# zyc00/Point-SAM

Measured on AMD Instinct MI355X. Metric: point-clouds/sec (encode+1-prompt decode), higher is better.
Workload: dtype f32 (fp32 in/out/accumulate; large GEMMs as row-scaled 2-way fp16 split x 3 MFMA products, fp32-grade error)

## Files before the change

include/pointsam_hip.h:

```cpp
#ifndef POINTSAM_HIP_H
#define POINTSAM_HIP_H

#include <stddef.h>
#include <stdint.h>

#ifdef __cplusplus
extern "C" {
#endif

typedef struct ihipStream_t* psam_stream_t;

#define PSAM_OK 0
#define PSAM_EINVAL (-1)
#define PSAM_EALIGN (-2)
#define PSAM_EWORKSPACE (-3)

#define PSAM_ACT_NONE 0
#define PSAM_ACT_GELU 1
#define PSAM_ACT_RELU 2
#define PSAM_ACT_SWIGLU 3

int32_t psam_version(void);
const char* psam_last_error_string(void);

// ... 59 lines not shown
void psam_gemm_f16x3p_force_splitk_fixup(int32_t mode);
#ifdef PSAM_BUILD_EXPERIMENTS
void psam_gemm_f16x3p_force_continuous(int32_t mode);
#endif
#define PSAM_COUNTER_BYTES 65536
void psam_attention_f16x3_force_keysplit(int32_t mode);
int32_t psam_attention_f16x3_last_instance(void);
int32_t psam_attention_f16x3_last_keysplit(void);
int32_t psam_attention_f32_last_instance(void);
#ifdef PSAM_BUILD_EXPERIMENTS
void psam_twoway_decoder_force_fork(int32_t mode);
#endif
int32_t psam_gemm_f16x3p_fused_row_ln(int32_t N);
typedef struct {
    float* out_scale; float out_k1, out_k2; int32_t pack_out;
    float* stats; int32_t stat_cols;
    const float* ln_mean; const float* ln_rstd; const float* ln_c;
    float* gmax_out; int64_t gmax_ld; int32_t gmax_k; int32_t no_store;
    const float* row_ln_g; const float* row_ln_b; float row_ln_eps;
    const float* hyper; float* masks; int32_t hyper_c; int32_t hyper_rows;
    int64_t hyper_pstride;
    float* splitk_ws; int64_t splitk_plane; int32_t splitk;
    const float* out_bound;
    int32_t* counters;
} psam_gemm_fuse_t;
int32_t psam_gemm_f16x3p_splitk(int32_t M, int32_t N, int32_t K, int32_t act);
int32_t psam_gemm_f16x3p_hyper_planes(int32_t N, int32_t with_row_ln);
int32_t psam_sum_planes(const float* parts, int32_t P, int64_t pstride, int64_t count, float* out, psam_stream_t stream);
int32_t psam_gemm_f16x3p_stat_segs(int32_t N);
int32_t psam_gemm_f16x3p_ex(const void* A, int64_t lda, const float* scaleA, const void* W, int64_t ldw, const float* scaleW, float* C, int64_t ldc,
                            const float* bias, const float* residual, int64_t ldr, const float* rowbias, int64_t ldrb, int32_t rowgroup, int32_t M,
                            int32_t N, int32_t K, float alpha, int32_t act, const psam_gemm_fuse_t* fuse, psam_stream_t stream);
int32_t psam_ln_stats_finalize(const float* stats, int32_t rows, int32_t segs, int32_t cols, float eps, float* mean, float* rstd, psam_stream_t stream);
int32_t psam_scale_pack_rows_g8(const float* X, int64_t ldx, int32_t rows, int32_t K, void* P, int64_t ldp, float* scale, psam_stream_t stream);
int32_t psam_linear(const float* x, int64_t ldx, const float* W, int64_t ldw, const float* bias, const float* residual, int64_t ldr, float* y,
                    int64_t ldy, int32_t M, int32_t N, int32_t K, int32_t act, psam_stream_t stream);
void psam_gemm_bf16x6_force_config(int32_t cfg);
void psam_gemm_force_config(int32_t cfg);

int32_t psam_layernorm(const float* x, int64_t ldx, const float* res, int64_t ldr, const float* w, const float* b, float* y, int64_t ldy,
                       int64_t rows, int32_t cols, float eps, int32_t act, psam_stream_t stream);
int32_t psam_layernorm_ex(const float* x, int64_t ldx, const float* res, int64_t ldr, const float* w, const float* b, float* y, int64_t ldy,
                          int64_t rows, int32_t cols, float eps, int32_t act, float* row_scale, int32_t pack, psam_stream_t stream);
int32_t psam_layernorm_ex2(const float* x, int64_t ldx, const float* res, int64_t ldr, const float* w, const float* b, float* y, int64_t ldy,
                           int64_t rows, int32_t cols, float eps, int32_t act, float* row_scale, int32_t pack, float* row_bound, float c2,
                           float c1, float c0, psam_stream_t stream);
int32_t psam_layernorm_rs(const float* x, int64_t ldx, const float* res, int64_t ldr, const float* w, const float* b, float* y, int64_t ldy,
                          int64_t rows, int32_t cols, float eps, int32_t act, float* row_scale, psam_stream_t stream);
int32_t psam_layernorm_last_instance(void);

int32_t psam_swiglu_ln(const float* gx, int64_t ldg, int32_t xoff, const float* w, const float* b, float* out, int64_t ldo, int64_t rows,
                       int32_t H, float eps, psam_stream_t stream);
int32_t psam_swiglu_ln_last_instance(void);

int32_t psam_attention_f32(const float* q, int64_t ldq, int64_t sq, const float* k, int64_t ldk, int64_t sk, const float* v, int64_t ldv,
                           int64_t sv, float* o, int64_t ldo, int64_t so, int32_t B, int32_t H, int32_t Lq, int32_t Lk, int32_t hd,
                           float scale, psam_stream_t stream);
int32_t psam_attention_f16x3(const float* q, int64_t ldq, int64_t sq, const float* k, int64_t ldk, int64_t sk, const float* v, int64_t ldv,
                           int64_t sv, float* o, int64_t ldo, int64_t so, int32_t B, int32_t H, int32_t Lq, int32_t Lk, int32_t hd,
                           float scale, psam_stream_t stream);
int32_t psam_attention_f16x3_ex(const float* q, int64_t ldq, int64_t sq, const float* k, int64_t ldk, int64_t sk, const float* v, int64_t ldv,
                                int64_t sv, float* o, int64_t ldo, int64_t so, int32_t B, int32_t H, int32_t Lq, int32_t Lk, int32_t hd, float scale,
                                const float* a_scale, float k1, float k2, float* o_scale, psam_stream_t stream);
size_t psam_attention_f16x3_keysplit_ws_bytes(int32_t B, int32_t H, int32_t Lq, int32_t Lk, int32_t hd, int32_t max_keysplit);
int32_t psam_attention_f16x3_ex2(const float* q, int64_t ldq, int64_t sq, const float* k, int64_t ldk, int64_t sk, const float* v, int64_t ldv,
                                int64_t sv, float* o, int64_t ldo, int64_t so, int32_t B, int32_t H, int32_t Lq, int32_t Lk, int32_t hd, float scale,
// ... 291 lines not shown
```

point_sam_amd/_lib.py:

```python
import ctypes
import os

_HERE = os.path.dirname(os.path.abspath(__file__))
LIB_PATH = os.environ.get("PSAM_HIP_LIB") or os.path.join(_HERE, "csrc", "libpointsam_hip.so")

i32, i64, f32 = ctypes.c_int32, ctypes.c_int64, ctypes.c_float
ptr, size_t = ctypes.c_void_p, ctypes.c_size_t

SIGNATURES = {
    "psam_version": (i32, []),
    "psam_last_error_string": (ctypes.c_char_p, []),
    "psam_fps_workspace_bytes": (size_t, [i32, i32, i32]),
    "psam_fps_set_cooperative": (None, [i32]),
    "psam_fps_set_pruning": (None, [i32]),
    "psam_fps": (i32, [ptr, i32, i32, i32, ptr, ptr, ptr, size_t, ptr]),
    "psam_knn": (i32, [ptr, ptr, i32, i32, i32, i32, ptr, ptr]),
    "psam_fps_last_instance": (i32, []),
    "psam_fps_last_grid_x": (i32, []),
    "psam_knn_force_band": (None, [i32]),
    "psam_knn_last_instance": (i32, []),
    "psam_three_nn": (i32, [ptr, ptr, i32, i32, i32, f32, ptr, ptr, ptr]),
    "psam_group_gather": (i32, [ptr, ptr, ptr, ptr, i32, i32, i32, i32, i32, i32, ptr, ptr]),
    "psam_group_gather_r": (i32, [ptr, ptr, ptr, ptr, i32, i32, i32, i32, i32, i32, f32, ptr, ptr]),
    "psam_group_gather_ld": (i32, [ptr, ptr, ptr, ptr, i32, i32, i32, i32, i32, i32, f32, ptr, i64, ptr]),
    "psam_patch_l1": (i32, [ptr, ptr, ptr, ptr, ptr, ptr, ptr, ptr, f32, i32, i32, i32, i32, i32, i32, ptr, ptr]),
    "psam_patch_l1_r": (i32, [ptr, ptr, ptr, ptr, ptr, ptr, ptr, ptr, f32, i32, i32, i32, i32, i32, i32, f32, ptr, ptr]),
    "psam_patch_l1_ex": (i32, [ptr, ptr, ptr, ptr, ptr, ptr, ptr, ptr, ptr, f32, i32, i32, i32, i32, i32, i32, f32, ptr, ptr, ptr]),
    "psam_error_regions": (i32, [ptr, ptr, ptr, ptr, i64, ptr]),
    "psam_border_farthest_workspace_bytes": (size_t, [i32, i32]),
    "psam_border_farthest": (i32, [ptr, ptr, i32, i32, i32, ptr, ptr, ptr, size_t, ptr]),
    "psam_group_max": (i32, [ptr, i64, ptr, i64, i64, i32, i32, ptr]),
    "psam_gemm_f32": (i32, [ptr, i64, i64, i64, ptr, i64, i64, i64, ptr, i64, i64, i64, ptr, ptr, i64, i64, i64, ptr, i64, i32,
                            i32, i32, i32, i32, i32, f32, i32, ptr]),
    "psam_gemm_bf16x6": (i32, [ptr, i64, i64, i64, ptr, i64, i64, i64, ptr, i64, i64, i64, ptr, ptr, i64, i64, i64, ptr, i64, i32,
                               i32, i32, i32, i32, i32, f32, i32, ptr]),
    "psam_linear": (i32, [ptr, i64, ptr, i64, ptr, ptr, i64, ptr, i64, i32, i32, i32, i32, ptr]),
    "psam_gemm_force_config": (None, [i32]),
    "psam_gemm_bf16x6_force_config": (None, [i32]),
    "psam_row_scale_f16": (i32, [ptr, i64, i32, i32, ptr, ptr]),
    "psam_pack_rows_f16x2_g8": (i32, [ptr, i64, ptr, i32, i32, ptr, i64, ptr]),
    "psam_gemm_f16x3p": (i32, [ptr, i64, ptr, ptr, i64, ptr, ptr, i64, ptr, ptr, i64, ptr, i64, i32, i32, i32, i32, f32, i32, ptr]),
    "psam_gemm_f16x3p_force_config": (None, [i32]),
    "psam_gemm_f16x3p_last_config": (i32, []),
    "psam_gemm_f16x3p_last_splitk": (i32, []),
    "psam_gemm_f16x3p_force_epilogue": (None, [i32]),
    "psam_gemm_f16x3p_force_splitk_fixup": (None, [i32]),
    "psam_gemm_f16x3p_force_continuous": (None, [i32]),
    "psam_attention_f16x3_force_keysplit": (None, [i32]),
    "psam_attention_f16x3_last_instance": (i32, []),
    "psam_attention_f16x3_last_keysplit": (i32, []),
    "psam_attention_f32_last_instance": (i32, []),
    "psam_twoway_decoder_force_fork": (None, [i32]),
    "psam_attention_packed_force_variant": (None, [i32]),
    "psam_attention_packed_force_nw": (None, [i32]),
    "psam_attention_packed_last_instance": (i32, []),
    "psam_gemm_f16x3p_fused_row_ln": (i32, [i32]),
    "psam_gemm_f16x3p_stat_segs": (i32, [i32]),
    "psam_gemm_f16x3p_splitk": (i32, [i32, i32, i32, i32]),
    "psam_nn_group_feats": (i32, [ptr, ptr, ptr, ptr, ptr, i32, i32, i32, i32, i32, i32, ptr, i64, ptr]),
    "psam_scatter_amax": (i32, [ptr, i64, ptr, i64, i32, i64, i64, i32, ptr, i64, i32, ptr]),
    "psam_eva_block_prepared_bytes": (size_t, [i32, i32]),
    "psam_eva_block_prepare": (i32, [ptr, ptr, ptr, size_t, ptr]),
    "psam_eva_block_ws_bytes": (size_t, [i64, i32, i32]),
    "psam_eva_block": (i32, [ptr, ptr, ptr, i32, i32, ptr, size_t, ptr]),
    "psam_linear_skinny_multi": (i32, [ptr, i64, i64, i64, i32, i32, ptr]),
    "psam_linear_skinny_ln": (i32, [ptr, i64, ptr, i64, ptr, ptr, i64, ptr, ptr, f32, ptr, ptr, i64, i32, i32, i32, ptr, ptr]),
    "psam_linear_rows_multi": (i32, [ptr, i64, i64, i32, i32, i64, i64, i32, ptr]),
    "psam_linear_ln256": (i32, [ptr, i64, ptr, i64, ptr, ptr, i64, ptr, ptr, f32, ptr, i64, i64, i32, i32, ptr]),
    "psam_twoway_decoder_force_fast": (None, [i32]),
    "psam_scale_pack_rows_g8_add_dual": (i32, [ptr, i64, ptr, i64, i32, i32, i32, i32, ptr, ptr, ptr, ptr, i64, ptr]),
    "psam_mlp3_pair": (i32, [ptr, ptr, i32, ptr]),
    "psam_attention_small_force_split": (None, [i32]),
    "psam_attention_small_last_instance": (i32, []),
    "psam_layernorm_last_instance": (i32, []),
    "psam_swiglu_ln_last_instance": (i32, []),
    "psam_patch_l1_last_instance": (i32, []),
    "psam_interp3_last_instance": (i32, []),
    "psam_linear_skinny_ln_tmp_floats": (ctypes.c_size_t, [i32, i32]),
    "psam_scale_pack_rows_g8_add": (i32, [ptr, i64, ptr, i64, i32, i32, i32, i32, ptr, i64, ptr, ptr]),
    "psam_eva_gelu_block_prepared_bytes": (size_t, [i32, i32]),
    "psam_eva_gelu_block_prepare": (i32, [ptr, ptr, ptr, size_t, ptr]),
    "psam_eva_gelu_block_ws_bytes": (size_t, [i64, i32, i32]),
    "psam_eva_gelu_block": (i32, [ptr, ptr, ptr, i32, i32, ptr, size_t, ptr, ptr]),
    "psam_patch_encoder_prepared_bytes": (size_t, [i32, i32, i32]),
    "psam_patch_encoder_prepare": (i32, [ptr, ptr, ptr, size_t, ptr]),
    "psam_patch_encoder_ws_bytes": (size_t, [i64, i64, i32, i32]),
    "psam_patch_encoder": (i32, [ptr, ptr, ptr, ptr, ptr, ptr, ptr, i32, i32, i32, i32, i32, i32, f32, ptr, ptr, size_t, ptr]),
    "psam_upscale_masks_prepared_bytes": (size_t, [i32]),
    "psam_upscale_masks_prepare": (i32, [ptr, ptr, ptr, size_t, ptr]),
# ... 211 lines not shown
```

point_sam_amd/build.py:

```python
import os
import subprocess
import sys
from concurrent.futures import ThreadPoolExecutor

CSRC = os.path.join(os.path.dirname(os.path.abspath(__file__)), "csrc")
LIB = os.path.join(CSRC, "libpointsam_hip.so")
HIPCC = os.environ.get("HIPCC", "/opt/rocm/bin/hipcc")
ARCH = "gfx950"
COMMON = ["--offload-arch=" + ARCH, "-O3", "-std=c++17", "-fPIC", "-fvisibility=hidden", "-Wall", "-Wno-unused-function"]
EXPERIMENTS = os.environ.get("PSAM_BUILD_EXPERIMENTS", "0") == "1"
SOURCES = [
    ("tokenizer.hip", ["-ffp-contract=off"]),
    ("gemm.hip", []),
    ("gemm_split.hip", []),
    ("gemm_f16x3p.hip", []),
    ("gemm_f16x3pp.hip", []),
    ("attention.hip", []),
    ("rowops.hip", []),
    ("blocks.hip", []),
    ("masks.hip", []),
    ("scene.hip", ["-ffp-contract=off"]),
    ("regions.hip", ["-ffp-contract=off"]),
    ("crops.hip", ["-ffp-contract=off"]),
    ("scene_interp.hip", ["-ffp-contract=off"]),
    ("transfer.hip", ["-ffp-contract=off", "-fno-slp-vectorize"]),
    ("align.hip", ["-ffp-contract=off", "-fno-slp-vectorize"]),
    ("views.hip", ["-ffp-contract=off", "-fno-slp-vectorize"]),
    ("frames.hip", ["-ffp-contract=off", "-fno-slp-vectorize"]),
    ("fusion.hip", ["-ffp-contract=off", "-fno-slp-vectorize"]),
    ("geometry.hip", ["-ffp-contract=off", "-fno-slp-vectorize"]),
    ("error.cpp", ["-x", "hip"]),
] + ([("experiments/gemm_f16x3q.hip", ["-I" + CSRC]), ("experiments/gemm_f16x3s.hip", ["-I" + CSRC]), ("experiments/gemm_f16x3c.hip", ["-I" + CSRC]),
        ("experiments/twoway.hip", ["-I" + CSRC])] if EXPERIMENTS else [])
if EXPERIMENTS:
    COMMON = COMMON + ["-DPSAM_BUILD_EXPERIMENTS"]
FLAGS_STAMP = os.path.join(CSRC, ".build_flags")
PROBE_SRC = os.path.join(CSRC, "probe", "mfma_probe.hip")
PROBE_LIB = os.path.join(CSRC, "probe", "libpsam_probe.so")


def _stale(out, deps):
    return not os.path.exists(out) or any(os.path.getmtime(d) > os.path.getmtime(out) for d in deps)


def build_library(force: bool = False, verbose: bool = False) -> str:
    hdrs = [os.path.join(CSRC, f) for f in sorted(os.listdir(CSRC)) if f.endswith(".h")]
    hdrs.append(os.path.join(os.path.dirname(os.path.dirname(CSRC)), "include", "pointsam_hip.h"))
    flags = " ".join(COMMON)
    if (open(FLAGS_STAMP).read() != flags) if os.path.exists(FLAGS_STAMP) else EXPERIMENTS:
# ... 41 lines not shown
```

point_sam_amd/csrc/blocks.hip:

```cpp
#include <algorithm>
#include <cmath>
#include <cstring>
#include <initializer_list>
#ifdef PSAM_BUILD_EXPERIMENTS
#include <map>
#include <mutex>
#endif
#include <string>
#include <utility>
#include <vector>
#include "g8_pack.h"

namespace {
constexpr int64_t align256(int64_t b) { return (b + 255) / 256 * 256; }

struct Carve {
    char* base; int64_t off = 0;
    explicit Carve(void* p) : base(static_cast<char*>(p)) {}
    template <typename T> T* take(int64_t count) { T* r = base ? reinterpret_cast<T*>(base + off) : nullptr; off += align256(count * (int64_t)sizeof(T)); return r; }
    int64_t offset_of(const void* p) const { return static_cast<const char*>(p) - base; }
};
template <typename F> size_t carved_bytes(F&& layout) { Carve cv(nullptr); layout(cv); return (size_t)cv.off; }

struct Packed { float* w; float* s; };
// ... 416 lines not shown
PSAM_API int32_t psam_patch_encoder(const psam_patch_encoder_plan_t* plan, const void* prepared, const float* xyz, const float* feats, const float* centers,
                                    const int64_t* knn_idx, const int64_t* center_idx, int32_t B, int32_t rep, int32_t N, int32_t G, int32_t K, int32_t C,
                                    float radius, float* out, void* ws, size_t ws_bytes, hipStream_t stream) {
    PSAM_REQUIRE(plan && prepared && xyz && feats && centers && knn_idx && out && ws, PSAM_EINVAL, "psam_patch_encoder: null pointer");
    const int h0 = plan->h0, h1 = plan->h1, cout = plan->cout, a = kpad32(h0), b = kpad32(h1);
    const int64_t groups = (int64_t)B * rep * G, rows = groups * K;
    PSAM_REQUIRE(B > 0 && rep > 0 && N > 0 && G > 0 && (K == 32 || (K > 0 && K % 64 == 0)) && rows % 256 == 0 && rows < ((int64_t)1 << 31), PSAM_EINVAL,
                 "psam_patch_encoder: group size must be 32 or a multiple of 64, and B * rep * G * K a multiple of 256");
    const int Kp = K <= 64 ? K : 64, parts = K / Kp;
    PSAM_REQUIRE(plan->cin == 3 + C * (center_idx ? 2 : 1), PSAM_EINVAL, "psam_patch_encoder: feature channels do not match the first Linear");
    PSAM_REQUIRE(ws_bytes >= psam_patch_encoder_ws_bytes(rows, groups, h0, h1), PSAM_EWORKSPACE, "psam_patch_encoder: workspace too small");
    auto P = [&](int64_t off) { return at(prepared, off); };
    Carve cv(ws);
    const PatchWs w = patch_ws(cv, rows, groups, h0, h1);
    float* part1 = parts > 1 ? w.x3 : w.y1;
    float* part2 = parts > 1 ? w.x1 : out;
    PSAM_REQUIRE(parts == 1 || ((int64_t)groups * parts * h0 <= rows * b && (int64_t)groups * parts * cout <= rows * a), PSAM_EINVAL,
                 "psam_patch_encoder: partial maxima do not fit the workspace");
    int32_t rc = psam_patch_l1_ex(xyz, feats, centers, knn_idx, center_idx, plan->c10_w, plan->c10_b, plan->c11_w, plan->c11_b, plan->eps, B, rep, N, G, K, C, radius, w.x1, w.s1, stream);
    if (rc) return rc;
    psam_gemm_fuse_t f;
    std::memset(&f, 0, sizeof(f));
    f.pack_out = 1; f.out_scale = w.s2; f.out_k1 = plan->k1; f.out_k2 = plan->k2; f.gmax_out = part1; f.gmax_ld = h0; f.gmax_k = Kp;
    rc = psam_gemm_f16x3p_ex(w.x1, a, w.s1, P(plan->o_w13), a, P(plan->o_s13), w.x2, a, plan->c13_b, nullptr, 0, nullptr, 0, 0, (int32_t)rows, h0, a, 1.f, 0, &f, stream);
    if (rc) return rc;
    if (parts > 1) { rc = psam_group_max(part1, h0, w.y1, h0, groups, parts, h0, stream); if (rc) return rc; }
    const Lin c20m{plan->c20_w, 2 * h0, plan->c20_b, P(plan->o_w20m), P(plan->o_s20m), h1, h0};
    rc = host_linear(c20m, w.y1, groups, w.g1, 0, G, w.y1p, w.sy, stream);
    if (rc) return rc;
    if (h1 == 512 && rows % 128 == 0 && psam_gemm_f16x3p_fused_row_ln(h1)) {
        std::memset(&f, 0, sizeof(f));
        f.row_ln_g = plan->c21_w; f.row_ln_b = plan->c21_b; f.row_ln_eps = plan->eps; f.pack_out = 1; f.out_scale = w.rs; f.out_k1 = 0.f; f.out_k2 = plan->ln21_bound;
        rc = psam_gemm_f16x3p_ex(w.x2, a, w.s2, P(plan->o_w20x), a, P(plan->o_s20x), w.x3, b, nullptr, nullptr, 0, w.g1, h1, K, (int32_t)rows, h1, a, 1.f, PSAM_ACT_GELU, &f, stream);
        if (rc) return rc;
    } else {
        rc = psam_gemm_f16x3p_ex(w.x2, a, w.s2, P(plan->o_w20x), a, P(plan->o_s20x), w.x3, h1, nullptr, nullptr, 0, w.g1, h1, K, (int32_t)rows, h1, a, 1.f, 0, nullptr, stream);
        if (rc) return rc;
        rc = psam_layernorm_ex(w.x3, h1, nullptr, 0, plan->c21_w, plan->c21_b, w.x3, b, rows, h1, plan->eps, PSAM_ACT_GELU, w.rs, 1, stream);
        if (rc) return rc;
    }
    std::memset(&f, 0, sizeof(f));
    f.gmax_out = part2; f.gmax_ld = cout; f.gmax_k = Kp; f.no_store = 1;
    rc = psam_gemm_f16x3p_ex(w.x3, b, w.rs, P(plan->o_w23), b, P(plan->o_s23), out, cout, plan->c23_b, nullptr, 0, nullptr, 0, 0, (int32_t)rows, cout, b, 1.f, 0, &f, stream);
    if (rc || parts == 1) return rc;
    return psam_group_max(part2, cout, out, cout, groups, parts, cout, stream);
}

namespace {
struct UpscalePrepared { Packed u0, u3; };
UpscalePrepared upscale_prepared(Carve& cv, int dim) { return {take_packed(cv, dim, dim), take_packed(cv, dim, dim)}; }

struct UpscaleWs { float *kp, *k1, *sk, *up, *s1, *parts; };
UpscaleWs upscale_ws(Carve& cv, int64_t Z, int N, int G, int C, int dim) {
    const int64_t a = kpad32(dim), planes = psam_gemm_f16x3p_hyper_planes(dim, 0);
    UpscaleWs w;
    w.kp = cv.take<float>(Z * G * a); w.k1 = cv.take<float>(Z * G * a); w.sk = cv.take<float>(Z * G);
    w.up = cv.take<float>(Z * N * a); w.s1 = cv.take<float>(Z * N);
    w.parts = cv.take<float>(planes * Z * C * N);
    return w;
}
}

PSAM_API size_t psam_upscale_masks_prepared_bytes(int32_t dim) {
    if (dim <= 0) return 0;
    return carved_bytes([&](Carve& cv) { upscale_prepared(cv, dim); });
}
// ... 404 lines not shown
```

point_sam_amd/csrc/g8_pack.h:

```cpp
#pragma once
#include "common.h"

typedef unsigned u32x4 __attribute__((ext_vector_type(4)));

static inline __host__ __device__ int kpad32(int k) { return (k + 31) & ~31; }

#ifdef __HIPCC__
typedef float psam_f32x2 __attribute__((ext_vector_type(2)));
typedef float psam_f32x4 __attribute__((ext_vector_type(4)));
typedef _Float16 psam_f16x2 __attribute__((ext_vector_type(2)));

__device__ __forceinline__ void g8_split2_scaled(const psam_f32x2 xs, unsigned& hi, unsigned& lo) {
    const psam_f16x2 h = __builtin_convertvector(xs, psam_f16x2);
    const psam_f32x2 r = xs - __builtin_convertvector(h, psam_f32x2);
    hi = __builtin_bit_cast(unsigned, h);
    lo = __builtin_bit_cast(unsigned, __builtin_convertvector(r, psam_f16x2));
}
__device__ __forceinline__ void psam_split2_f16(float x0, float x1, float s, unsigned& hi, unsigned& lo) { g8_split2_scaled(psam_f32x2{x0, x1} * s, hi, lo); }

__device__ __forceinline__ float g8_absmax4(const psam_f32x4 v) { return fmaxf(fmaxf(fabsf(v[0]), fabsf(v[1])), fmaxf(fabsf(v[2]), fabsf(v[3]))); }
__device__ __forceinline__ float g8_absmax4(float amax, const psam_f32x4 v) { return fmaxf(fmaxf(amax, fmaxf(fabsf(v[0]), fabsf(v[1]))), fmaxf(fabsf(v[2]), fabsf(v[3]))); }
__device__ __forceinline__ float g8_row_scale(float lane_max) { return f16_row_scale(wave_max(lane_max)); }

template <int DIST, bool SHFL = false>
// ... 17 lines not shown
    unsigned h0, l0, h1, l1;
    psam_split2_f16(x[0], x[1], s, h0, l0);
    psam_split2_f16(x[2], x[3], s, h1, l1);
    return g8_chunk_words<DIST, SHFL>(h0, l0, h1, l1, lane);
}
template <int DIST>
__device__ __forceinline__ u32x4 g8_chunk_scaled(const psam_f32x2 xs01, const psam_f32x2 xs23, int lane) {
    unsigned h0, l0, h1, l1;
    g8_split2_scaled(xs01, h0, l0);
    g8_split2_scaled(xs23, h1, l1);
    return g8_chunk_words<DIST>(h0, l0, h1, l1, lane);
}

struct g8_group { u32x4 hi, lo; };
__device__ __forceinline__ g8_group g8_halfwave_group(const psam_f32x4 x, const psam_f32x4 y, float s) {
    unsigned xh[2], xl[2], yh[2], yl[2];
    psam_split2_f16(x[0], x[1], s, xh[0], xl[0]);
    psam_split2_f16(x[2], x[3], s, xh[1], xl[1]);
    psam_split2_f16(y[0], y[1], s, yh[0], yl[0]);
    psam_split2_f16(y[2], y[3], s, yh[1], yl[1]);
    psam_swap32(xh[0], yh[0]); psam_swap32(xh[1], yh[1]); psam_swap32(xl[0], yl[0]); psam_swap32(xl[1], yl[1]);
    return {u32x4{xh[0], xh[1], yh[0], yh[1]}, u32x4{xl[0], xl[1], yl[0], yl[1]}};
}
__device__ __forceinline__ g8_group g8_whole_group(const float (&v)[8], float s) {
    unsigned hi[4], lo[4];
#pragma unroll
    for (int e = 0; e < 4; ++e) psam_split2_f16(v[2 * e], v[2 * e + 1], s, hi[e], lo[e]);
    return {u32x4{hi[0], hi[1], hi[2], hi[3]}, u32x4{lo[0], lo[1], lo[2], lo[3]}};
}
__device__ __forceinline__ void g8_store_group(unsigned* first, const g8_group& g) {
    *reinterpret_cast<u32x4*>(first) = g.hi;
    *reinterpret_cast<u32x4*>(first + 4) = g.lo;
}

__device__ __forceinline__ void g8_store_pair(unsigned* P, int64_t row, int ld, int lane, float x0, float x1, float s) {
    unsigned hi, lo;
    psam_split2_f16(x0, x1, s, hi, lo);
    unsigned* o = P + row * ld + (lane >> 2) * 8 + (lane & 3);
    o[0] = hi;
    o[4] = lo;
}
#endif
```

point_sam_amd/model.py:

```python
import math
from dataclasses import dataclass, field
from types import SimpleNamespace
from typing import Optional

import torch

from . import ops
from .config import ModelConfig
from .ops import ACT_GELU, ACT_NONE, ACT_RELU
from .streams import pipeline_streams
from .weights import check_state_dict


def _round_up(x, m):
    return (x + m - 1) // m * m


@dataclass
class TokenizerState:
    fps_idx: torch.Tensor
    centers: torch.Tensor
    knn_idx: torch.Tensor
    interp_index: torch.Tensor
    interp_weight: torch.Tensor
# ... 185 lines not shown
        h0 = self.cfg.patch_hidden[0]
        rows = feats.shape[0] * knn_idx.shape[1] * K
        l1 = (w[prefix + ".conv1.0.weight"], w[prefix + ".conv1.0.bias"], w[prefix + ".conv1.1.weight"], w[prefix + ".conv1.1.bias"], eps)
        w2a = w[prefix + ".conv2.0.weight"]
        fused = (self.precision == "f16x3" and self.fuse_patch and (K in (32, 64) or K % 64 == 0) and ops.fuse_supported(rows, 128) and prefix in self.pe_bound
                 and all((prefix + n) in self.fw for n in (".conv1.3.weight", ".conv2.0.weight#x", ".conv2.3.weight")))
        if fused and self.c_blocks and prefix in getattr(self, "c_patch", {}) and ops.current_gemm_mode() == "f16x3":
            return self.c_patch[prefix].run(coords, feats, centers, knn_idx, radius=radius, center_idx=center_idx)
        if fused:
            groups = rows // K
            s1 = torch.empty(rows, dtype=torch.float32, device=coords.device)
            h1 = ops.patch_l1(coords, feats, centers, knn_idx, *l1, radius=radius, center_idx=center_idx, scale_out=s1)
            h2 = torch.empty(rows, h0, dtype=torch.float32, device=coords.device)
            s2 = torch.empty(rows, dtype=torch.float32, device=coords.device)
            Kp = K if K <= 64 else 64
            parts = K // Kp
            y1 = torch.empty(groups * parts, h0, dtype=torch.float32, device=coords.device)
            k1, k2 = self.pe_bound[prefix]
            self._lin(prefix + ".conv1.3", h1, x_scale=s1, x_packed=True, out=h2, pack_out=(s2, k1, k2), group_max_out=y1, group_max_k=Kp)
            if parts > 1:
                y1 = ops.group_max(y1, parts)
            del h1
            g1 = ops.linear(y1, self.fw.get(prefix + ".conv2.0.weight#max", w2a[:, :h0]), w[prefix + ".conv2.0.bias"])
            hd1 = w2a.shape[0]
            if ops.fused_row_ln(hd1) and hd1 == 512 and (prefix + ".conv2.3.weight") in self.fw and rows % 128 == 0:
                h3 = torch.empty(rows, hd1, dtype=torch.float32, device=coords.device)
                rs, pk = torch.empty(rows, dtype=torch.float32, device=coords.device), True
                bound = self.ln_bound.get(prefix)
                if bound is None:
                    bound = self.ln_bound.setdefault(prefix, 1.001 * ops.row_ln_bound(w[prefix + ".conv2.1.weight"], w[prefix + ".conv2.1.bias"]) + 1e-30)
                ops.linear(h2, self.fw[prefix + ".conv2.0.weight#x"], None, act=ACT_GELU, rowbias=g1, rowgroup=K, x_scale=s2, x_packed=True, out=h3,
                           row_ln=(w[prefix + ".conv2.1.weight"], w[prefix + ".conv2.1.bias"], eps), pack_out=(rs, 0.0, bound))
                del h2
            else:
                h3 = ops.linear(h2, self.fw[prefix + ".conv2.0.weight#x"], None, rowbias=g1, rowgroup=K, x_scale=s2, x_packed=True)
                del h2
                pk, rs = self._ln_feeds_gemm(h3, prefix + ".conv2.3")
                self._ln(prefix + ".conv2.1", h3, eps, act=ACT_GELU, out=h3, scale_out=rs, pack=pk)
            emb = torch.empty(groups * parts, self.w[prefix + ".conv2.3.weight"].shape[0], dtype=torch.float32, device=coords.device)
            self._lin(prefix + ".conv2.3", h3, x_scale=rs, x_packed=pk, group_max_out=emb, group_max_k=Kp, no_store=True)
            return ops.group_max(emb, parts) if parts > 1 else emb
        h1 = ops.patch_l1(coords, feats, centers, knn_idx, *l1, radius=radius, center_idx=center_idx)
        h2 = self._lin(prefix + ".conv1.3", h1)
        del h1
        y1 = ops.group_max(h2, K)
        g1 = ops.linear(y1, self.fw.get(prefix + ".conv2.0.weight#max", w2a[:, :h0]), w[prefix + ".conv2.0.bias"])
        h3 = ops.linear(h2, self.fw.get(prefix + ".conv2.0.weight#x", w2a[:, h0:]), None, rowbias=g1, rowgroup=K)
        del h2
        pk, rs = self._ln_feeds_gemm(h3, prefix + ".conv2.3")
        self._ln(prefix + ".conv2.1", h3, eps, act=ACT_GELU, out=h3, scale_out=rs, pack=pk)
        h4 = self._lin(prefix + ".conv2.3", h3, x_scale=rs, x_packed=pk)
        del h3
        return ops.group_max(h4, K)

    def _block(self, blk, x, B, L):
        vit = self.cfg.vit
        D, H, hd = vit.dim, vit.heads, vit.head_dim
        p = blk.p
        f16 = self.precision == "f16x3"
        if (f16 and self.c_blocks and hasattr(blk, "c_block") and self.fuse_mlp and self.fuse_attn_pack and self.fuse_attn_operands
                and self.row_bounds and ops.current_gemm_mode() == "f16x3" and x.is_contiguous()
                and (x.shape[0] % 256 == 0 if vit.swiglu else x.shape[0] >= ops.SPLIT_MIN_M)):
            return blk.c_block.run(x, B, L)
        pk = f16 and x.shape[0] >= ops.SPLIT_MIN_M and isinstance(blk.wqkv, ops.F16Weight) and ops.layernorm_can_pack(D)
        rs = torch.empty(x.shape[0], dtype=torch.float32, device=x.device) if pk else None
        h = self._ln(p + ".norm1", x, vit.ln_eps, scale_out=rs, pack=pk)
# ... 519 lines not shown
```

point_sam_amd/ops.py:

```python
import ctypes
import torch

from . import _lib
from ._lib import check

ACT_NONE, ACT_GELU, ACT_RELU, ACT_SWIGLU = 0, 1, 2, 3

GEMM_PROFILE = None
GEMM_PROFILE_EVERY = 29
GEMM_PROFILE_OTHERS = ()
GEMM_PROFILE_AFTER = 0
_gemm_counter = 0


def _sample_now():
    return GEMM_PROFILE is not None and _gemm_counter > GEMM_PROFILE_AFTER and _gemm_counter % GEMM_PROFILE_EVERY == 0


def _sampled_launch(launch, record):
    cur = torch.cuda.current_stream()
    for o in GEMM_PROFILE_OTHERS:
        cur.wait_stream(o)
    s, e = torch.cuda.Event(enable_timing=True), torch.cuda.Event(enable_timing=True)
    s.record()
# ... 322 lines not shown
    global _gemm_counter
    import ctypes
    L = _lib.load()
    _gemm_counter += 1
    fn_args = fn_args[:-1] + (ctypes.byref(fuse) if fuse is not None else None, fn_args[-1])
    if not _sample_now():
        check(L.psam_gemm_f16x3p_ex(*fn_args), "psam_gemm_f16x3p")
        return
    _sampled_launch(lambda: check(L.psam_gemm_f16x3p_ex(*fn_args), "psam_gemm_f16x3p"), lambda s, e: GEMM_PROFILE.append((s, e, flops, M, N, K, "f16x3")))


_SPLITK = {}


def splitk_factor(M: int, N: int, K: int, act: int) -> int:
    key = (M, N, K, act, torch.cuda.current_device())
    ks = _SPLITK.get(key)
    if ks is None:
        ks = _SPLITK[key] = int(_lib.load().psam_gemm_f16x3p_splitk(M, N, K, act))
    return ks


def fuse_supported(M: int, N: int) -> bool:
    return M % 256 == 0 and N % 128 == 0


def row_ln_bound(gamma, beta) -> float:
    n = gamma.numel()
    return float((n - 1) ** 0.5 * gamma.abs().max().item() + beta.abs().max().item())


def fused_row_ln(N: int) -> bool:
    return bool(_lib.load().psam_gemm_f16x3p_fused_row_ln(int(N)))


def stat_segs(N: int) -> int:
    return (N // 2 + 31) // 32


def ln_stats_finalize(stats, cols, eps):
    M, segs, _ = stats.shape
    mean = torch.empty(M, dtype=torch.float32, device=stats.device)
    rstd = torch.empty(M, dtype=torch.float32, device=stats.device)
    check(_lib.load().psam_ln_stats_finalize(stats.data_ptr(), M, segs, cols, eps, mean.data_ptr(), rstd.data_ptr(), _stream()), "psam_ln_stats_finalize")
    return mean, rstd


def linear(x, W, bias=None, act=ACT_NONE, residual=None, out=None, rowbias=None, rowgroup=0, K=None, x_scale=None, x_packed=False,
           pack_out=None, stats=None, ln_fold=None, group_max_out=None, group_max_k=0, no_store=False, row_ln=None, hyper=None):
    fw = None
    if isinstance(W, F16Weight):
        fw, W = W, W.fp32
    xp, ldx = _row_view(x, "x")
    wp, ldw = _row_view(W, "W")
    M = x.shape[0]
    N = W.shape[0]
    if K is None:
        K = W.shape[1]
        assert x_packed or x.shape[1] == K, (x.shape, W.shape)
    elif fw is not None and K != fw.K:
        fw = None
    fused = pack_out is not None or stats is not None or ln_fold is not None or group_max_out is not None or row_ln is not None or hyper is not None
    if no_store and (group_max_out is not None or hyper is not None) and out is None:
        op, ldo = (group_max_out if group_max_out is not None else hyper[1]).data_ptr(), N
    else:
        if out is None:
# ... 1497 lines not shown
```

Before: 818.8.

## Fuse patch conv2 K=128 GEMM with row LayerNorm, GELU and fp16 pack

Adds a dedicated kernel for the patch-embedding conv2.0 GEMM when K=128 and N=512. A block of eight waves covers a full 512-column row, so the LayerNorm, GELU and packed fp16x2 output for conv2.3 are computed in registers. It keeps weights resident in registers, double-buffers input tiles via buffer DMA, and loops persistently over row blocks. This removes the separate GEMM output write plus the LN/pack pass and their reads, at the cost of a specialised kernel with high register pressure and fixed shape requirements.

Result: faster. 827.4, median of 6 (+1.1%).

```diff
diff --git a/include/pointsam_hip.h b/include/pointsam_hip.h
--- a/include/pointsam_hip.h
+++ b/include/pointsam_hip.h
@@ -115,6 +115,9 @@
                             const float* bias, const float* residual, int64_t ldr, const float* rowbias, int64_t ldrb, int32_t rowgroup, int32_t M,
                             int32_t N, int32_t K, float alpha, int32_t act, const psam_gemm_fuse_t* fuse, psam_stream_t stream);
 int32_t psam_ln_stats_finalize(const float* stats, int32_t rows, int32_t segs, int32_t cols, float eps, float* mean, float* rstd, psam_stream_t stream);
+int32_t psam_linear128_ln_gelu_pack(const void* x, int64_t ldx, const float* x_scale, const void* w, int64_t ldw, const float* w_scale, const float* rowbias,
+                                    int64_t ldrb, int32_t rowgroup, const float* gamma, const float* beta, float eps, float bound, int64_t rows, int32_t h1,
+                                    void* out, int64_t ldo, float* out_scale, psam_stream_t stream);
 int32_t psam_scale_pack_rows_g8(const float* X, int64_t ldx, int32_t rows, int32_t K, void* P, int64_t ldp, float* scale, psam_stream_t stream);
 int32_t psam_linear(const float* x, int64_t ldx, const float* W, int64_t ldw, const float* bias, const float* residual, int64_t ldr, float* y,
                     int64_t ldy, int32_t M, int32_t N, int32_t K, int32_t act, psam_stream_t stream);
diff --git a/point_sam_amd/_lib.py b/point_sam_amd/_lib.py
--- a/point_sam_amd/_lib.py
+++ b/point_sam_amd/_lib.py
@@ -55,6 +55,7 @@
     "psam_attention_packed_force_nw": (None, [i32]),
     "psam_attention_packed_last_instance": (i32, []),
     "psam_gemm_f16x3p_fused_row_ln": (i32, [i32]),
+    "psam_linear128_ln_gelu_pack": (i32, [ptr, i64, ptr, ptr, i64, ptr, ptr, i64, i32, ptr, ptr, f32, f32, i64, i32, ptr, i64, ptr, ptr]),
     "psam_gemm_f16x3p_stat_segs": (i32, [i32]),
     "psam_gemm_f16x3p_splitk": (i32, [i32, i32, i32, i32]),
     "psam_nn_group_feats": (i32, [ptr, ptr, ptr, ptr, ptr, i32, i32, i32, i32, i32, i32, ptr, i64, ptr]),
diff --git a/point_sam_amd/build.py b/point_sam_amd/build.py
--- a/point_sam_amd/build.py
+++ b/point_sam_amd/build.py
@@ -15,6 +15,7 @@
     ("gemm_split.hip", []),
     ("gemm_f16x3p.hip", []),
     ("gemm_f16x3pp.hip", []),
+    ("patch_rowln.hip", []),
     ("attention.hip", []),
     ("rowops.hip", []),
     ("blocks.hip", []),
diff --git a/point_sam_amd/csrc/blocks.hip b/point_sam_amd/csrc/blocks.hip
--- a/point_sam_amd/csrc/blocks.hip
+++ b/point_sam_amd/csrc/blocks.hip
@@ -472,6 +472,10 @@
         std::memset(&f, 0, sizeof(f));
         f.row_ln_g = plan->c21_w; f.row_ln_b = plan->c21_b; f.row_ln_eps = plan->eps; f.pack_out = 1; f.out_scale = w.rs; f.out_k1 = 0.f; f.out_k2 = plan->ln21_bound;
         rc = psam_gemm_f16x3p_ex(w.x2, a, w.s2, P(plan->o_w20x), a, P(plan->o_s20x), w.x3, b, nullptr, nullptr, 0, w.g1, h1, K, (int32_t)rows, h1, a, 1.f, PSAM_ACT_GELU, &f, stream);
+        if (rc) return rc;
+    } else if (h0 == 128 && h1 == 512 && rows % 64 == 0) {
+        rc = psam_linear128_ln_gelu_pack(w.x2, a, w.s2, P(plan->o_w20x), a, P(plan->o_s20x), w.g1, h1, K, plan->c21_w, plan->c21_b, plan->eps, plan->ln21_bound, rows, h1,
+                                         w.x3, b, w.rs, stream);
         if (rc) return rc;
     } else {
         rc = psam_gemm_f16x3p_ex(w.x2, a, w.s2, P(plan->o_w20x), a, P(plan->o_s20x), w.x3, h1, nullptr, nullptr, 0, w.g1, h1, K, (int32_t)rows, h1, a, 1.f, 0, nullptr, stream);
diff --git a/point_sam_amd/csrc/g8_pack.h b/point_sam_amd/csrc/g8_pack.h
--- a/point_sam_amd/csrc/g8_pack.h
+++ b/point_sam_amd/csrc/g8_pack.h
@@ -73,6 +73,7 @@
     *reinterpret_cast<u32x4*>(first) = g.hi;
     *reinterpret_cast<u32x4*>(first + 4) = g.lo;
 }
+__device__ __forceinline__ void g8_store_halfwave_group(unsigned* first, const psam_f32x4 x, const psam_f32x4 y, float s) { g8_store_group(first, g8_halfwave_group(x, y, s)); }
 
 __device__ __forceinline__ void g8_store_pair(unsigned* P, int64_t row, int ld, int lane, float x0, float x1, float s) {
     unsigned hi, lo;
diff --git a/point_sam_amd/csrc/patch_rowln.hip b/point_sam_amd/csrc/patch_rowln.hip
--- /dev/null
+++ b/point_sam_amd/csrc/patch_rowln.hip
@@ -0,0 +1,212 @@
+#include "g8_pack.h"
+#include "gemm_f16x3p_args.h"
+#include "gemm_epilogue_t.h"
+
+namespace {
+struct RowLnArgs {
+    const unsigned char* X; const unsigned char* W;
+    const float* sx; const float* sw;
+    const float* rowbias; const float* gamma; const float* beta;
+    unsigned* out; float* rs;
+    int64_t ldx, ldw, ldrb, ldo;
+    int rowgroup, nblocks;
+    float eps, bound;
+};
+
+constexpr int RL_ROWS = 64, RL_K = 128, RL_N = 512, RL_WAVES = 8;
+constexpr int RL_ROWB = 128;
+constexpr int RL_SLAB = RL_ROWS * RL_ROWB;
+constexpr int RL_STAGE = (RL_K / 32) * RL_SLAB;
+
+__device__ __forceinline__ void rl_barrier() { asm volatile("s_waitcnt lgkmcnt(0)\n\ts_barrier" ::: "memory"); }
+
+__global__ __launch_bounds__(64 * RL_WAVES) void linear128_ln_gelu_pack_kernel(const RowLnArgs p) {
+#pragma clang fp contract(off)
+    __shared__ __attribute__((aligned(16))) unsigned char stage_mem[2 * RL_STAGE];
+    __shared__ float red[2 * RL_WAVES * RL_ROWS];
+    __shared__ __attribute__((aligned(16))) float cst[3 * RL_N];
+    __shared__ __attribute__((aligned(16))) float rbs[2 * 2 * RL_N];
+    const int tid = threadIdx.x, lane = tid & 63;
+    const int wave = __builtin_amdgcn_readfirstlane(tid >> 6);
+    const int col_base = wave * 64;
+
+    const int drow = wave * 8 + (lane >> 3);
+    const int dvoff = (int)(drow * p.ldx * 4) + (((lane & 7) ^ ((drow >> 1) & 7)) << 4);
+    auto issue = [&](int blk, int st) {
+        const __amdgpu_buffer_rsrc_t rs = __builtin_amdgcn_make_buffer_rsrc((void*)(p.X + (int64_t)blk * RL_ROWS * p.ldx * 4), 0, 0x7fffffff, 0x00020000);
+#pragma unroll
+        for (int s = 0; s < RL_K / 32; ++s) P_DMA16(rs, stage_mem + st * RL_STAGE + s * RL_SLAB + wave * 1024, dvoff, s * RL_ROWB);
+    };
+    int blk = blockIdx.x, st = 0;
+    issue(blk, 0);
+
+    pf16x8 fw[2][8][2];
+    {
+        const unsigned char* wl = p.W + (int64_t)(col_base + (lane & 31)) * p.ldw * 4 + (lane >> 5) * 32;
+#pragma unroll
+        for (int j = 0; j < 2; ++j)
+#pragma unroll
+            for (int ks = 0; ks < 8; ++ks)
+#pragma unroll
+                for (int q = 0; q < 2; ++q) fw[j][ks][q] = *reinterpret_cast<const pf16x8*>(wl + (int64_t)j * 32 * p.ldw * 4 + ks * 64 + q * 16);
+    }
+    const float so = f16_row_scale(p.bound);
+    const float inv_n = 1.0f / (float)RL_N;
+    float* red2 = red + RL_WAVES * RL_ROWS;
+    cst[tid] = inv_pow2(p.sw[tid]); cst[RL_N + tid] = p.gamma[tid]; cst[2 * RL_N + tid] = p.beta[tid];
+    auto bias_fetch = [&](int b, float (&v)[2]) {
+#pragma unroll
+        for (int i = 0; i < 2; ++i) v[i] = p.rowbias[(int64_t)((b * RL_ROWS + i * 32) / p.rowgroup) * p.ldrb + tid];
+    };
+    {
+        float v[2];
+        bias_fetch(blk, v);
+        rbs[tid] = v[0]; rbs[RL_N + tid] = v[1];
+    }
+
+    asm volatile("s_waitcnt vmcnt(0)" ::: "memory");
+    rl_barrier();
+    for (; blk < p.nblocks; blk += gridDim.x, st ^= 1) {
+        const bool has_next = blk + (int)gridDim.x < p.nblocks;
+        if (has_next) issue(blk + gridDim.x, st ^ 1);
+        const int64_t row0 = (int64_t)blk * RL_ROWS;
+        const unsigned char* sa = stage_mem + st * RL_STAGE;
+        if (wave == 0) p.rs[row0 + lane] = so;
+        const float sxv = p.sx[row0 + lane];
+        int lf = lane;
+        asm volatile("" : "+v"(lf));
+        int fa_off[2][2];
+#pragma unroll
+        for (int s = 0; s < 2; ++s)
+#pragma unroll
+            for (int q = 0; q < 2; ++q) fa_off[s][q] = (lf & 31) * RL_ROWB + (((4 * s + 2 * (lf >> 5) + q) ^ ((lf >> 1) & 7)) << 4);
+        pf32x16 acc[2][2];
+#pragma unroll
+        for (int i = 0; i < 2; ++i)
+#pragma unroll
+            for (int j = 0; j < 2; ++j)
+#pragma unroll
+                for (int r = 0; r < 16; ++r) acc[i][j][r] = 0.f;
+#pragma unroll
+        for (int ks = 0; ks < 8; ++ks) {
+            pf16x8 fa[2][2];
+#pragma unroll
+            for (int i = 0; i < 2; ++i)
+#pragma unroll
+                for (int q = 0; q < 2; ++q) fa[i][q] = *reinterpret_cast<const pf16x8*>(sa + (ks >> 1) * RL_SLAB + i * 32 * RL_ROWB + fa_off[ks & 1][q]);
+            constexpr int PA[3] = {0, 1, 0}, PW[3] = {1, 0, 0};
+#pragma unroll
+            for (int t = 0; t < 3; ++t)
+#pragma unroll
+                for (int i = 0; i < 2; ++i)
+#pragma unroll
+                    for (int j = 0; j < 2; ++j) acc[i][j] = __builtin_amdgcn_mfma_f32_32x32x16_f16(fw[j][ks][PW[t]], fa[i][PA[t]], acc[i][j], 0, 0, 0);
+            ept_fence();
+        }
+        int ln = lane;
+        asm volatile("" : "+v"(ln));
+        const int r32 = ln & 31, h = ln >> 5;
+        const int ccol = col_base + 4 * h;
+        float nb[2];
+        bias_fetch(has_next ? blk + gridDim.x : blk, nb);
+        const float rsq[2] = {inv_pow2(__shfl(sxv, r32, 64)), inv_pow2(__shfl(sxv, 32 + r32, 64))};
+        float sum[2] = {0.f, 0.f};
+        const float* rbl = rbs + st * 2 * RL_N + ccol;
+#pragma unroll
+        for (int n = 0; n < 8; ++n) {
+            const int j = n >> 2, g = n & 3;
+            if ((n & 1) == 0) ept_fence();
+            const ep_f32x4 isw = ep_load4(cst + ccol + 8 * n), rb[2] = {ep_load4(rbl + 8 * n), ep_load4(rbl + RL_N + 8 * n)};
+#pragma unroll
+            for (int i = 0; i < 2; ++i)
+#pragma unroll
+                for (int e = 0; e < 4; ++e) {
+                    const float a = (acc[i][j][4 * g + e] * rsq[i]) * isw[e] + rb[i][e];
+                    acc[i][j][4 * g + e] = a;
+                    sum[i] += a;
+                }
+        }
+        float mean[2], rstd[2];
+#pragma unroll
+        for (int i = 0; i < 2; ++i) {
+            float a = sum[i], b = sum[i];
+            ept_swap32f(a, b);
+            sum[i] = h == 0 ? a + b : b + a;
+            red[wave * RL_ROWS + i * 32 + r32] = sum[i];
+        }
+        rl_barrier();
+#pragma unroll
+        for (int i = 0; i < 2; ++i) {
+            float t = 0.f;
+#pragma unroll
+            for (int w = 0; w < RL_WAVES; ++w) t += red[w * RL_ROWS + i * 32 + r32];
+            mean[i] = t * inv_n;
+        }
+#pragma unroll
+        for (int i = 0; i < 2; ++i) {
+            float q = 0.f;
+#pragma unroll
+            for (int j = 0; j < 2; ++j) {
+                ept_fence();
+#pragma unroll
+                for (int r = 0; r < 16; ++r) { const float d = acc[i][j][r] - mean[i]; q = __builtin_fmaf(d, d, q); }
+            }
+            float a = q, b = q;
+            ept_swap32f(a, b);
+            q = h == 0 ? a + b : b + a;
+            red2[wave * RL_ROWS + i * 32 + r32] = q;
+        }
+        rbs[(st ^ 1) * 2 * RL_N + tid] = nb[0]; rbs[(st ^ 1) * 2 * RL_N + RL_N + tid] = nb[1];
+        asm volatile("s_waitcnt vmcnt(0)" ::: "memory");
+        rl_barrier();
+#pragma unroll
+        for (int i = 0; i < 2; ++i) {
+            float t = 0.f;
+#pragma unroll
+            for (int w = 0; w < RL_WAVES; ++w) t += red2[w * RL_ROWS + i * 32 + r32];
+            rstd[i] = 1.0f / sqrtf(t * inv_n + p.eps);
+        }
+        unsigned* ob = p.out + row0 * p.ldo + col_base + 8 * h;
+#pragma unroll
+        for (int j = 0; j < 2; ++j)
+#pragma unroll
+            for (int gp = 0; gp < 2; ++gp) {
+                const float* gb = cst + RL_N + ccol + j * 32 + 16 * gp;
+                const ep_f32x4 gm0 = ep_load4(gb), gm1 = ep_load4(gb + 8), bt0 = ep_load4(gb + RL_N), bt1 = ep_load4(gb + RL_N + 8);
+#pragma unroll
+                for (int i = 0; i < 2; ++i) {
+                    ep_f32x4 v0, v1;
+                    ept_fence();
+#pragma unroll
+                    for (int e = 0; e < 4; ++e) v0[e] = gelu_erf(__builtin_fmaf((acc[i][j][8 * gp + e] - mean[i]) * rstd[i], gm0[e], bt0[e]));
+                    ept_fence();
+#pragma unroll
+                    for (int e = 0; e < 4; ++e) v1[e] = gelu_erf(__builtin_fmaf((acc[i][j][8 * gp + 4 + e] - mean[i]) * rstd[i], gm1[e], bt1[e]));
+                    g8_store_halfwave_group(ob + (int64_t)(i * 32 + r32) * p.ldo + j * 32 + 16 * gp, v0, v1, so);
+                }
+            }
+    }
+}
+}
+
+PSAM_API int32_t psam_linear128_ln_gelu_pack(const void* x, int64_t ldx, const float* x_scale, const void* w, int64_t ldw, const float* w_scale, const float* rowbias,
+                                             int64_t ldrb, int32_t rowgroup, const float* gamma, const float* beta, float eps, float bound, int64_t rows, int32_t h1,
+                                             void* out, int64_t ldo, float* out_scale, hipStream_t stream) {
+#define WHO "psam_linear128_ln_gelu_pack"
+    PSAM_REQUIRE(x && x_scale && w && w_scale && rowbias && gamma && beta && out && out_scale, PSAM_EINVAL, WHO ": null pointer");
+    PSAM_REQUIRE(h1 == RL_N, PSAM_EINVAL, WHO ": the output rows must have 512 columns");
+    PSAM_REQUIRE(rows > 0 && rows % RL_ROWS == 0 && rows < ((int64_t)1 << 31), PSAM_EINVAL, WHO ": rows must be a positive multiple of 64 below 2^31");
+    PSAM_REQUIRE(rowgroup > 0 && rowgroup % 32 == 0 && ldx >= RL_K && ldw >= RL_K && ldrb >= RL_N && ldo >= RL_N && ldx * 4 * RL_ROWS < ((int64_t)1 << 31), PSAM_EINVAL,
+                 WHO ": bad shape (packed inputs of 128 containers per row, bias and output rows of 512, a bias row per multiple of 32 rows)");
+    PSAM_REQUIRE(((ldx | ldw | ldo) & 7) == 0 && (((uintptr_t)x | (uintptr_t)w | (uintptr_t)out) & 31) == 0, PSAM_EALIGN, WHO ": packed rows must be 32-byte aligned");
+    PSAM_REQUIRE((ldrb & 3) == 0 && (((uintptr_t)rowbias | (uintptr_t)gamma | (uintptr_t)beta | (uintptr_t)w_scale) & 15) == 0, PSAM_EALIGN,
+                 WHO ": bias rows, gamma, beta and the weight's scales must be 16-byte aligned");
+    RowLnArgs p;
+    p.X = (const unsigned char*)x; p.W = (const unsigned char*)w; p.sx = x_scale; p.sw = w_scale; p.rowbias = rowbias; p.gamma = gamma; p.beta = beta;
+    p.out = (unsigned*)out; p.rs = out_scale; p.ldx = ldx; p.ldw = ldw; p.ldrb = ldrb; p.ldo = ldo; p.rowgroup = rowgroup; p.nblocks = (int)(rows / RL_ROWS);
+    p.eps = eps; p.bound = bound;
+    const int grid = p.nblocks < 2 * psam_cu_count() ? p.nblocks : 2 * psam_cu_count();
+    hipLaunchKernelGGL(linear128_ln_gelu_pack_kernel, dim3((unsigned)grid), dim3(64 * RL_WAVES), 0, stream, p);
+    return psam_launch_status(WHO ": launch failed");
+#undef WHO
+}
diff --git a/point_sam_amd/model.py b/point_sam_amd/model.py
--- a/point_sam_amd/model.py
+++ b/point_sam_amd/model.py
@@ -241,6 +241,15 @@
                 ops.linear(h2, self.fw[prefix + ".conv2.0.weight#x"], None, act=ACT_GELU, rowbias=g1, rowgroup=K, x_scale=s2, x_packed=True, out=h3,
                            row_ln=(w[prefix + ".conv2.1.weight"], w[prefix + ".conv2.1.bias"], eps), pack_out=(rs, 0.0, bound))
                 del h2
+            elif ops.linear128_ln_gelu_supported(rows, h0, hd1, K) and (prefix + ".conv2.3.weight") in self.fw and ops.current_gemm_mode() == "f16x3":
+                h3 = torch.empty(rows, hd1, dtype=torch.float32, device=coords.device)
+                rs, pk = torch.empty(rows, dtype=torch.float32, device=coords.device), True
+                bound = self.ln_bound.get(prefix)
+                if bound is None:
+                    bound = self.ln_bound.setdefault(prefix, 1.001 * ops.row_ln_bound(w[prefix + ".conv2.1.weight"], w[prefix + ".conv2.1.bias"]) + 1e-30)
+                ops.linear128_ln_gelu_pack(h2, s2, self.fw[prefix + ".conv2.0.weight#x"], g1, K, w[prefix + ".conv2.1.weight"], w[prefix + ".conv2.1.bias"], eps, bound,
+                                           h3, rs)
+                del h2
             else:
                 h3 = ops.linear(h2, self.fw[prefix + ".conv2.0.weight#x"], None, rowbias=g1, rowgroup=K, x_scale=s2, x_packed=True)
                 del h2
diff --git a/point_sam_amd/ops.py b/point_sam_amd/ops.py
--- a/point_sam_amd/ops.py
+++ b/point_sam_amd/ops.py
@@ -378,6 +378,20 @@
 
 def fused_row_ln(N: int) -> bool:
     return bool(_lib.load().psam_gemm_f16x3p_fused_row_ln(int(N)))
+
+
+def linear128_ln_gelu_supported(rows: int, K: int, N: int, rowgroup: int) -> bool:
+    return K == 128 and N == 512 and rows > 0 and rows % 64 == 0 and rowgroup > 0 and rowgroup % 32 == 0
+
+
+def linear128_ln_gelu_pack(x, x_scale, fw, rowbias, rowgroup, gamma, beta, eps, bound, out, scale_out):
+    xp, ldx = _row_view(x, "x")
+    rbp, ldrb = _row_view(rowbias, "rowbias")
+    op, ldo = _row_view(out, "out")
+    check(_lib.load().psam_linear128_ln_gelu_pack(xp, ldx, x_scale.data_ptr(), fw.packed.data_ptr(), fw.packed.stride(0), fw.scale.data_ptr(), rbp, ldrb, int(rowgroup),
+                                                  gamma.data_ptr(), beta.data_ptr(), float(eps), float(bound), x.shape[0], fw.N, op, ldo,
+                                                  scale_out.data_ptr(), _stream()), "psam_linear128_ln_gelu_pack")
+    return out
 
 
 def stat_segs(N: int) -> int:
```
